# fperezgamonal/flownet2-tf

Hardware: AMD Instinct MI355X
Metric: forward pairs/sec at 512x384 (FlowNet2) (higher is better)
Workload: dtype f16x2 (split fp16 hi+lo operands, 3 fp16 MFMAs per product, fp32 accumulate); 1 GPU; FlowNet2 forward, batch=4 synthetic 512x384 pairs per GPU, seeded synthetic weights; pairs_per_gpu=4, parallelism=dp1 (no collective)

## Files before the change

### flownet2-tf_amd/csrc/corr3.hip

```cpp
#include "fn2_common.h"

namespace fn2 {

typedef __attribute__((address_space(3))) void* lptr3_t;

struct CorrArgs {
  const void* a;
  const void* b;
  void* out;
  int N, H, W;
  int a_cs, a_c0, b_cs, b_c0, out_cs, out_c0;
  int md, s2, gr, gw, lo;
  int act;
  float c_f;
};

#ifndef FN2_C3_XS
#define FN2_C3_XS 2
#endif
constexpr int C3_XS = FN2_C3_XS;
constexpr int C3_HALF = C3_XS == 2 ? 64 : 48;
constexpr int C3_ROWS = 2 * C3_HALF;
constexpr int C3_OTS = 168;
#ifndef FN2_C3_SLOTS
#define FN2_C3_SLOTS 3
#endif
constexpr int C3_SLOTS = FN2_C3_SLOTS;
constexpr int C3_SG = 1;
constexpr int C3_TY = 2;
constexpr int C3_NW = 2 * C3_TY * C3_XS;
constexpr int C3_PX = 32 * C3_TY * C3_XS;
constexpr unsigned kOob3 = 0x80000000u;

typedef int v4i3_t __attribute__((ext_vector_type(4)));

__device__ __forceinline__ void dma16_3(const v4i3_t rsrc, const void* lds, unsigned voff, int soff) {
  const unsigned la = (unsigned)(unsigned long long)(lptr3_t)lds;
  asm volatile("s_mov_b32 m0, %0\n\ts_nop 0\n\tbuffer_load_dwordx4 %1, %2, %3 offen lds"
               :: "s"(la), "v"(voff), "s"(rsrc), "s"(soff) : "memory");
}

template <typename T, typename OutT, int NL>
__global__ void __launch_bounds__(64 * C3_NW) corr3_kernel(const CorrArgs p, const int b_bytes, const int dbg) {
#if defined(__HIP_DEVICE_COMPILE__)
  constexpr int ESZ = (int)sizeof(T);
  constexpr bool X2 = is_x2<T>::value;
  constexpr int SG = NL < C3_SG ? 1 : C3_SG;
  constexpr int NST = NL / SG;
  constexpr int NPIECE = C3_ROWS * SG / 8;
  constexpr int PPW = (NPIECE + C3_NW - 1) / C3_NW;
  __shared__ uint4 ring[C3_SLOTS][C3_SG][C3_ROWS * 8];
  __shared__ float ot[C3_PX * C3_OTS];

  const int tid = threadIdx.x, lane = tid & 63;
  const int wave = __builtin_amdgcn_readfirstlane(tid >> 6);
  const int gx = gridDim.x, gy = gridDim.y;
  const int NT = gx * gy * (int)gridDim.z, L = blockIdx.x + gx * (blockIdx.y + gy * blockIdx.z);
  const int xcd = L & 7, chk = NT >> 3, rem = NT & 7;
  const int Lp = xcd * chk + min(xcd, rem) + (L >> 3);
  const int xb = (Lp % gx) * (32 * C3_XS);
  const int g = (Lp / gx) % gy;
  const int zc = Lp / (gx * gy);
  const int n = zc / 3, c = zc - n * 3;
  const int y0 = 2 * C3_TY * (g >> 1) + (g & 1);
  const int pi0 = 8 * c, npi = min(8, p.gw - pi0);

  const int fi = lane & 15, fg = lane >> 4;
  const int hh = wave % C3_XS, par = (wave / C3_XS) & 1, r = wave / (2 * C3_XS);
  const int ya = y0 + 2 * r;
  const int xa = xb + 32 * hh + par + 2 * fi;

  for (int i = tid; i < C3_PX * C3_OTS / 4; i += 64 * C3_NW) reinterpret_cast<float4*>(ot)[i] = make_float4(0.f, 0.f, 0.f, 0.f);

  uint4 fa[NL][2];
  {
    const bool ok = xa < p.W && ya < p.H;
    const char* src = reinterpret_cast<const char*>(p.a) +
                      ((((size_t)n * p.H + (ok ? ya : 0)) * p.W + (ok ? xa : 0)) * p.a_cs + p.a_c0) * ESZ;
#pragma unroll
    for (int l = 0; l < NL; ++l)
#pragma unroll
      for (int q = 0; q < 2; ++q) {
        const int chunk = X2 ? (2 * fg + q) : (4 * q + fg);
        fa[l][q] = ok ? *reinterpret_cast<const uint4*>(src + l * 128 + chunk * 16) : make_uint4(0, 0, 0, 0);
      }
  }

  const int yb0 = y0 + 2 * (pi0 - p.gr);
  int k_lo = 0, k_hi = npi + C3_TY - 2;
  while (k_lo <= k_hi && yb0 + 2 * k_lo < 0) ++k_lo;
  while (k_hi >= k_lo && yb0 + 2 * k_hi >= p.H) --k_hi;
  const int nrow = k_hi - k_lo + 1;
  const int S = nrow > 0 ? nrow * NST : 0;

  const v4i3_t rsrc = v4i3_t{(int)((unsigned long long)p.b & 0xffffffffu), (int)(((unsigned long long)p.b >> 32) & 0xffffu),
                             b_bytes, 0x00020000};
  unsigned voff[PPW];
#pragma unroll
  for (int k = 0; k < PPW; ++k) {
    const int q = wave * PPW + k;
    const int sl = q / (C3_ROWS / 8), rg = q - sl * (C3_ROWS / 8);
    const int rho = rg * 8 + (lane >> 3);
    const int Lc = (lane & 7) ^ ((rho >> 1) & 7);
    const int G = X2 ? ((Lc & 3) * 2 + (Lc >> 2)) : Lc;
    const int px = rho < C3_HALF ? 2 * rho : 2 * (rho - C3_HALF) + 1;
    const int xw = xb - p.md + px;
    const bool ok = q < NPIECE && xw >= 0 && xw < p.W;
    voff[k] = ok ? (unsigned)((xw * p.b_cs + p.b_c0) * ESZ + sl * 128 + G * 16) : kOob3;
  }
  const int row_bytes = p.W * p.b_cs * ESZ;
  int is_s = 0, is_st = 0, is_slot = 0;
  int is_soff = (n * p.H + yb0 + 2 * k_lo) * row_bytes;
  auto issue_stage = [&]() {
    uint4 (*slot)[C3_ROWS * 8] = ring[is_slot];
    const bool live = is_s < S;
#pragma unroll
    for (int k = 0; k < PPW; ++k) {
      const int q = wave * PPW + k;
      const int sl = q / (C3_ROWS / 8), rg = q - sl * (C3_ROWS / 8);
      if (q < NPIECE && !(dbg & 1)) dma16_3(rsrc, &slot[sl][rg * 64], live ? voff[k] : kOob3, live ? is_soff : 0);
    }
    ++is_s;
    is_slot = is_slot == C3_SLOTS - 1 ? 0 : is_slot + 1;
    if (++is_st == NST) { is_st = 0; is_soff += 2 * row_bytes - (NST - 1) * SG * 128; }
    else is_soff += SG * 128;
  };

  const int fsw = (fi >> 1) & 7;
  const int rbase = par * C3_HALF + 16 * hh + fi;
  const int ci = (int)p.c_f;
  const bool pow2 = (ci & (ci - 1)) == 0;
  const float rcp = 1.f / p.c_f;
  f32x4 acc[3];
#pragma unroll
  for (int tb = 0; tb < 3; ++tb) acc[tb] = f32x4{0.f, 0.f, 0.f, 0.f};

  if (S > 0) {
#pragma unroll
    for (int d = 0; d < C3_SLOTS - 1; ++d) issue_stage();
    __syncthreads();
    int cslot = 0;
    for (int kk = 0; kk < nrow; ++kk) {
#pragma unroll
      for (int st = 0; st < NST; ++st) {
        static_assert(PPW * (C3_SLOTS - 2) <= 63, "vmcnt field");
        asm volatile("s_waitcnt vmcnt(%0)\n\ts_barrier" :: "n"(PPW * (C3_SLOTS - 2)) : "memory");
        issue_stage();
        uint4 (*slot)[C3_ROWS * 8] = ring[cslot];
        cslot = cslot == C3_SLOTS - 1 ? 0 : cslot + 1;
        const int pil_s = k_lo + kk - r;
        if (!(dbg & 2) && pil_s >= 0 && pil_s < npi)
#pragma unroll
        for (int sl = 0; sl < SG; ++sl) {
          const int l = st * SG + sl;
#pragma unroll
          for (int tb = 0; tb < 3; ++tb) {
            const uint4* row = &slot[sl][(rbase + 16 * tb) * 8];
            const uint4 b0 = row[fg ^ fsw], b1 = row[(4 + fg) ^ fsw];
            if constexpr (X2) {
              acc[tb] = mfma_16x16x32<f16_t>(fa[l][1], b0, acc[tb]);
              acc[tb] = mfma_16x16x32<f16_t>(fa[l][0], b1, acc[tb]);
              acc[tb] = mfma_16x16x32<f16_t>(fa[l][0], b0, acc[tb]);
            } else {
              acc[tb] = mfma_16x16x32<T>(fa[l][0], b0, acc[tb]);
              acc[tb] = mfma_16x16x32<T>(fa[l][1], b1, acc[tb]);
            }
          }
        }
      }
      const int pil = k_lo + kk - r;
      const bool rowok = pil >= 0 && pil < npi;
#pragma unroll
      for (int tb = 0; tb < 3; ++tb) {
#pragma unroll
        for (int q = 0; q < 4; ++q) {
          const int i = fg * 4 + q;
          const int o = 16 * tb + fi - i;
          if (rowok && o >= 0 && o <= 2 * p.gr && !(dbg & 4)) {
            float v = pow2 ? acc[tb][q] * rcp : acc[tb][q] / p.c_f;
            if (p.act == FN2_ACT_LEAKY) v = leaky(v);
            ot[(r * 32 * C3_XS + 32 * hh + par + 2 * i) * C3_OTS + pil * p.gw + o] = v;
          }
        }
        acc[tb] = f32x4{0.f, 0.f, 0.f, 0.f};
      }
    }
    asm volatile("s_waitcnt vmcnt(0)" ::: "memory");
  }
  __syncthreads();

  if (dbg & 8) return;
  OutT* out = reinterpret_cast<OutT*>(p.out);
  const int nch = npi * p.gw;
  const int ch0 = p.out_c0 + pi0 * p.gw;
  if constexpr (is_x2<OutT>::value) {
    const int ngrp = nch >> 3;
    for (int idx = tid; idx < C3_PX * ngrp; idx += 64 * C3_NW) {
      const int px = idx / ngrp, gi = idx - px * ngrp;
      const int rr = px / (32 * C3_XS), x = xb + px % (32 * C3_XS), y = y0 + 2 * rr;
      if (x >= p.W || y >= p.H) continue;
      const float* src = &ot[px * C3_OTS + gi * 8];
      float v[8];
      *reinterpret_cast<float4*>(v) = *reinterpret_cast<const float4*>(src);
      *reinterpret_cast<float4*>(v + 4) = *reinterpret_cast<const float4*>(src + 4);
      uint4* q = reinterpret_cast<uint4*>(out + (((size_t)n * p.H + y) * p.W + x) * p.out_cs + ch0 + gi * 8);
      split8(v, q[0], q[1]);
    }
    const int tail = nch - (ngrp << 3);
    for (int idx = tid; idx < C3_PX * tail; idx += 64 * C3_NW) {
      const int px = idx / tail, j = (ngrp << 3) + (idx - px * tail);
      const int rr = px / (32 * C3_XS), x = xb + px % (32 * C3_XS), y = y0 + 2 * rr;
      if (x < p.W && y < p.H)
        store_elem<OutT>(out + (((size_t)n * p.H + y) * p.W + x) * p.out_cs + ch0 + j, ot[px * C3_OTS + j]);
    }
  } else {
    for (int idx = tid; idx < C3_PX * nch; idx += 64 * C3_NW) {
      const int px = idx / nch, j = idx - px * nch;
      const int rr = px / (32 * C3_XS), x = xb + px % (32 * C3_XS), y = y0 + 2 * rr;
      if (x < p.W && y < p.H)
        store_elem<OutT>(out + (((size_t)n * p.H + y) * p.W + x) * p.out_cs + ch0 + j, ot[px * C3_OTS + j]);
    }
  }
#endif
}

template <typename T, typename OutT>
static int launch3(const CorrArgs& a, int C, int b_bytes, hipStream_t s) {
  const int nl = C * (int)sizeof(T) / 128;
  dim3 grid(cdiv(a.W, 32 * C3_XS), a.H / C3_TY, a.N * 3), block(64 * C3_NW);
  const char* e_dbg = getenv("FN2_CORR3_DBG");
  const int dbg = e_dbg ? atoi(e_dbg) : 0;
  switch (nl) {
#define FN2_C3_CASE(NL_)                                                               \
  case NL_:                                                                            \
    hipLaunchKernelGGL((corr3_kernel<T, OutT, NL_>), grid, block, 0, s, a, b_bytes, dbg);   \
    break;
    FN2_C3_CASE(1)
    FN2_C3_CASE(2)
    FN2_C3_CASE(4)
    FN2_C3_CASE(8)
#undef FN2_C3_CASE
    default:
      return fail(FN2_ERR_UNSUPPORTED, "correlation: unsupported channel count %d", C);
  }
  FN2_CHECK_LAUNCH("corr3");
  return FN2_OK;
}

bool corr3_ok(int C, int in_dtype, int out_dtype, int md, int s2, int H, int out_cs, int out_c0, long b_bytes) {
  const char* e = getenv("FN2_CORR3");
  if (e && atoi(e) == 0) return false;
  if (in_dtype == FN2_F32) return false;
  const int esz = dtype_size(in_dtype);
  if ((C * esz) % 128 != 0) return false;
  const int nl = C * esz / 128;
  if (!(nl == 1 || nl == 2 || nl == 4 || nl == 8)) return false;
  if (md != 20 || s2 != 2 || H % (2 * C3_TY) != 0 || b_bytes >= (1L << 31)) return false;
  if (out_dtype == FN2_F16X2 && (out_cs % 8 != 0 || out_c0 % 8 != 0)) return false;
  return true;
}

int launch_corr3(const void* a, int a_cs, int a_c0, const void* b, int b_cs, int b_c0, void* out, int out_cs,
                 int out_c0, int in_dtype, int out_dtype, int N, int H, int W, int C, int md, int s2, int gr, int gw,
                 int act, hipStream_t s) {
  CorrArgs g;
  g.a = a; g.b = b; g.out = out;
  g.N = N; g.H = H; g.W = W;
  g.a_cs = a_cs; g.a_c0 = a_c0; g.b_cs = b_cs; g.b_c0 = b_c0; g.out_cs = out_cs; g.out_c0 = out_c0;
  g.md = md; g.s2 = s2; g.gr = gr; g.gw = gw; g.lo = md - gr * s2;
  g.act = act;
  g.c_f = (float)C;
  const int bb = (int)((long)N * H * W * b_cs * dtype_size(in_dtype));
  if (in_dtype == FN2_BF16) return out_dtype == FN2_BF16 ? launch3<bf16_t, bf16_t>(g, C, bb, s) : launch3<bf16_t, float>(g, C, bb, s);
  if (in_dtype == FN2_F16) return out_dtype == FN2_F16 ? launch3<f16_t, f16_t>(g, C, bb, s) : launch3<f16_t, float>(g, C, bb, s);
  return out_dtype == FN2_F16X2 ? launch3<x2_t, x2_t>(g, C, bb, s) : launch3<x2_t, float>(g, C, bb, s);
}

}
```

Before: 1131 pairs/s.

## Keep all correlation rows in registers and use per-wave LDS transpose epilogue

The correlation kernel now keeps accumulators for every displacement row in registers (acc[KR][3]) instead of flushing to a shared output tile after each row, and stages two channel slices per pipeline step. The shared ring and the output staging buffer are merged into one LDS array. Each wave transposes its own results through that buffer and writes them out without a block-wide barrier. Displacement radius is hardcoded to 10, and the scale and leaky branches are specialised at compile time. The aim is to cut LDS footprint, per-row epilogue work and block syncs, at the cost of much higher register pressure and reduced generality.

```diff
diff --git a/flownet2-tf_amd/csrc/corr3.hip b/flownet2-tf_amd/csrc/corr3.hip
--- a/flownet2-tf_amd/csrc/corr3.hip
+++ b/flownet2-tf_amd/csrc/corr3.hip
@@ -1,3 +1,5 @@
+#include <type_traits>
+
 #include "fn2_common.h"
 
 namespace fn2 {
@@ -15,21 +17,19 @@
   float c_f;
 };
 
-#ifndef FN2_C3_XS
-#define FN2_C3_XS 2
-#endif
-constexpr int C3_XS = FN2_C3_XS;
-constexpr int C3_HALF = C3_XS == 2 ? 64 : 48;
+constexpr int C3_XS = 2;
+constexpr int C3_HALF = 64;
 constexpr int C3_ROWS = 2 * C3_HALF;
-constexpr int C3_OTS = 168;
-#ifndef FN2_C3_SLOTS
-#define FN2_C3_SLOTS 3
-#endif
-constexpr int C3_SLOTS = FN2_C3_SLOTS;
-constexpr int C3_SG = 1;
+constexpr int C3_LINE = C3_ROWS * 8;
+constexpr int C3_GR = 10, C3_GW = 2 * C3_GR + 1;
+constexpr int C3_OTS = 8 * C3_GW;
+constexpr int C3_SLOTS = 3;
+constexpr int C3_SG = 2;
 constexpr int C3_TY = 2;
 constexpr int C3_NW = 2 * C3_TY * C3_XS;
-constexpr int C3_PX = 32 * C3_TY * C3_XS;
+constexpr int C3_KR = 8 + C3_TY - 1;
+constexpr int C3_PXS = 192, C3_ROW0 = 24;
+constexpr int C3_EPI = 16 * C3_PXS + 32;
 constexpr unsigned kOob3 = 0x80000000u;
 
 typedef int v4i3_t __attribute__((ext_vector_type(4)));
@@ -38,6 +38,11 @@
   const unsigned la = (unsigned)(unsigned long long)(lptr3_t)lds;
   asm volatile("s_mov_b32 m0, %0\n\ts_nop 0\n\tbuffer_load_dwordx4 %1, %2, %3 offen lds"
                :: "s"(la), "v"(voff), "s"(rsrc), "s"(soff) : "memory");
+}
+
+__device__ __forceinline__ float leaky_c3(float x) {
+#pragma clang fp contract(off)
+  return 0.55f * x + 0.45f * fabsf(x);
 }
 
 template <typename T, typename OutT, int NL>
@@ -45,12 +50,13 @@
 #if defined(__HIP_DEVICE_COMPILE__)
   constexpr int ESZ = (int)sizeof(T);
   constexpr bool X2 = is_x2<T>::value;
-  constexpr int SG = NL < C3_SG ? 1 : C3_SG;
+  constexpr int SG = NL < C3_SG ? NL : C3_SG;
   constexpr int NST = NL / SG;
   constexpr int NPIECE = C3_ROWS * SG / 8;
   constexpr int PPW = (NPIECE + C3_NW - 1) / C3_NW;
-  __shared__ uint4 ring[C3_SLOTS][C3_SG][C3_ROWS * 8];
-  __shared__ float ot[C3_PX * C3_OTS];
+  constexpr int RING16 = C3_SLOTS * SG * C3_LINE;
+  constexpr int EPI16 = C3_NW * C3_EPI / 4;
+  __shared__ uint4 lds[RING16 > EPI16 ? RING16 : EPI16];
 
   const int tid = threadIdx.x, lane = tid & 63;
   const int wave = __builtin_amdgcn_readfirstlane(tid >> 6);
@@ -63,14 +69,12 @@
   const int zc = Lp / (gx * gy);
   const int n = zc / 3, c = zc - n * 3;
   const int y0 = 2 * C3_TY * (g >> 1) + (g & 1);
-  const int pi0 = 8 * c, npi = min(8, p.gw - pi0);
+  const int pi0 = 8 * c, npi = min(8, C3_GW - pi0);
 
   const int fi = lane & 15, fg = lane >> 4;
   const int hh = wave % C3_XS, par = (wave / C3_XS) & 1, r = wave / (2 * C3_XS);
   const int ya = y0 + 2 * r;
   const int xa = xb + 32 * hh + par + 2 * fi;
-
-  for (int i = tid; i < C3_PX * C3_OTS / 4; i += 64 * C3_NW) reinterpret_cast<float4*>(ot)[i] = make_float4(0.f, 0.f, 0.f, 0.f);
 
   uint4 fa[NL][2];
   {
@@ -86,7 +90,7 @@
       }
   }
 
-  const int yb0 = y0 + 2 * (pi0 - p.gr);
+  const int yb0 = y0 + 2 * (pi0 - C3_GR);
   int k_lo = 0, k_hi = npi + C3_TY - 2;
   while (k_lo <= k_hi && yb0 + 2 * k_lo < 0) ++k_lo;
   while (k_hi >= k_lo && yb0 + 2 * k_hi >= p.H) --k_hi;
@@ -112,13 +116,13 @@
   int is_s = 0, is_st = 0, is_slot = 0;
   int is_soff = (n * p.H + yb0 + 2 * k_lo) * row_bytes;
   auto issue_stage = [&]() {
-    uint4 (*slot)[C3_ROWS * 8] = ring[is_slot];
+    uint4* slot = lds + is_slot * (SG * C3_LINE);
     const bool live = is_s < S;
 #pragma unroll
     for (int k = 0; k < PPW; ++k) {
       const int q = wave * PPW + k;
       const int sl = q / (C3_ROWS / 8), rg = q - sl * (C3_ROWS / 8);
-      if (q < NPIECE && !(dbg & 1)) dma16_3(rsrc, &slot[sl][rg * 64], live ? voff[k] : kOob3, live ? is_soff : 0);
+      if (q < NPIECE && !(dbg & 1)) dma16_3(rsrc, &slot[sl * C3_LINE + rg * 64], live ? voff[k] : kOob3, live ? is_soff : 0);
     }
     ++is_s;
     is_slot = is_slot == C3_SLOTS - 1 ? 0 : is_slot + 1;
@@ -128,97 +132,128 @@
 
   const int fsw = (fi >> 1) & 7;
   const int rbase = par * C3_HALF + 16 * hh + fi;
-  const int ci = (int)p.c_f;
-  const bool pow2 = (ci & (ci - 1)) == 0;
-  const float rcp = 1.f / p.c_f;
-  f32x4 acc[3];
-#pragma unroll
-  for (int tb = 0; tb < 3; ++tb) acc[tb] = f32x4{0.f, 0.f, 0.f, 0.f};
+  f32x4 acc[C3_KR][3];
+#pragma unroll
+  for (int k = 0; k < C3_KR; ++k)
+#pragma unroll
+    for (int tb = 0; tb < 3; ++tb) acc[k][tb] = f32x4{0.f, 0.f, 0.f, 0.f};
 
   if (S > 0) {
 #pragma unroll
     for (int d = 0; d < C3_SLOTS - 1; ++d) issue_stage();
-    __syncthreads();
+#pragma unroll
+    for (int l = 0; l < NL; ++l)
+#pragma unroll
+      for (int q = 0; q < 2; ++q) {
+        v4i3_t t = __builtin_bit_cast(v4i3_t, fa[l][q]);
+        asm volatile("" : "+v"(t));
+        fa[l][q] = __builtin_bit_cast(uint4, t);
+      }
     int cslot = 0;
-    for (int kk = 0; kk < nrow; ++kk) {
-#pragma unroll
-      for (int st = 0; st < NST; ++st) {
-        static_assert(PPW * (C3_SLOTS - 2) <= 63, "vmcnt field");
-        asm volatile("s_waitcnt vmcnt(%0)\n\ts_barrier" :: "n"(PPW * (C3_SLOTS - 2)) : "memory");
-        issue_stage();
-        uint4 (*slot)[C3_ROWS * 8] = ring[cslot];
-        cslot = cslot == C3_SLOTS - 1 ? 0 : cslot + 1;
-        const int pil_s = k_lo + kk - r;
-        if (!(dbg & 2) && pil_s >= 0 && pil_s < npi)
-#pragma unroll
-        for (int sl = 0; sl < SG; ++sl) {
-          const int l = st * SG + sl;
-#pragma unroll
-          for (int tb = 0; tb < 3; ++tb) {
-            const uint4* row = &slot[sl][(rbase + 16 * tb) * 8];
-            const uint4 b0 = row[fg ^ fsw], b1 = row[(4 + fg) ^ fsw];
+#pragma unroll
+    for (int k = 0; k < C3_KR; ++k) {
+      if (k >= k_lo && k <= k_hi) {
+        const int pil = k - r;
+        const bool used = !(dbg & 2) && pil >= 0 && pil < npi;
+#pragma unroll
+        for (int st = 0; st < NST; ++st) {
+          static_assert(PPW * (C3_SLOTS - 2) <= 63, "vmcnt field");
+          asm volatile("s_waitcnt vmcnt(%0)\n\ts_barrier" :: "n"(PPW * (C3_SLOTS - 2)) : "memory");
+          issue_stage();
+          const uint4* slot = lds + cslot * (SG * C3_LINE);
+          cslot = cslot == C3_SLOTS - 1 ? 0 : cslot + 1;
+          if (used)
+#pragma unroll
+          for (int sl = 0; sl < SG; ++sl) {
+            const int l = st * SG + sl;
+            uint4 b0[3], b1[3];
+#pragma unroll
+            for (int tb = 0; tb < 3; ++tb) {
+              const uint4* row = &slot[sl * C3_LINE + (rbase + 16 * tb) * 8];
+              b0[tb] = row[fg ^ fsw];
+              b1[tb] = row[(4 + fg) ^ fsw];
+            }
             if constexpr (X2) {
-              acc[tb] = mfma_16x16x32<f16_t>(fa[l][1], b0, acc[tb]);
-              acc[tb] = mfma_16x16x32<f16_t>(fa[l][0], b1, acc[tb]);
-              acc[tb] = mfma_16x16x32<f16_t>(fa[l][0], b0, acc[tb]);
+#pragma unroll
+              for (int tb = 0; tb < 3; ++tb) acc[k][tb] = mfma_16x16x32<f16_t>(fa[l][1], b0[tb], acc[k][tb]);
+#pragma unroll
+              for (int tb = 0; tb < 3; ++tb) acc[k][tb] = mfma_16x16x32<f16_t>(fa[l][0], b1[tb], acc[k][tb]);
+#pragma unroll
+              for (int tb = 0; tb < 3; ++tb) acc[k][tb] = mfma_16x16x32<f16_t>(fa[l][0], b0[tb], acc[k][tb]);
             } else {
-              acc[tb] = mfma_16x16x32<T>(fa[l][0], b0, acc[tb]);
-              acc[tb] = mfma_16x16x32<T>(fa[l][1], b1, acc[tb]);
+#pragma unroll
+              for (int tb = 0; tb < 3; ++tb) acc[k][tb] = mfma_16x16x32<T>(fa[l][0], b0[tb], acc[k][tb]);
+#pragma unroll
+              for (int tb = 0; tb < 3; ++tb) acc[k][tb] = mfma_16x16x32<T>(fa[l][1], b1[tb], acc[k][tb]);
             }
           }
         }
       }
-      const int pil = k_lo + kk - r;
-      const bool rowok = pil >= 0 && pil < npi;
-#pragma unroll
-      for (int tb = 0; tb < 3; ++tb) {
-#pragma unroll
-        for (int q = 0; q < 4; ++q) {
-          const int i = fg * 4 + q;
-          const int o = 16 * tb + fi - i;
-          if (rowok && o >= 0 && o <= 2 * p.gr && !(dbg & 4)) {
-            float v = pow2 ? acc[tb][q] * rcp : acc[tb][q] / p.c_f;
-            if (p.act == FN2_ACT_LEAKY) v = leaky(v);
-            ot[(r * 32 * C3_XS + 32 * hh + par + 2 * i) * C3_OTS + pil * p.gw + o] = v;
+    }
+    asm volatile("s_waitcnt vmcnt(0)" ::: "memory");
+    __syncthreads();
+  }
+
+  float* ow = reinterpret_cast<float*>(lds) + wave * C3_EPI;
+  auto transpose = [&](auto pow2_c, auto leaky_c) {
+    constexpr bool POW2 = decltype(pow2_c)::value, LEAKY = decltype(leaky_c)::value;
+    const float rcp = 1.f / p.c_f;
+    float* wb = ow + 4 * fg * (C3_PXS - 1) + fi + C3_ROW0 - r * C3_GW;
+#pragma unroll
+    for (int tb = 0; tb < 3; ++tb)
+#pragma unroll
+      for (int q = 0; q < 4; ++q) {
+        const int o = 16 * tb + fi - (fg * 4 + q);
+        if (o >= 0 && o <= 2 * C3_GR)
+#pragma unroll
+          for (int k = 0; k < C3_KR; ++k) {
+            float v = POW2 ? acc[k][tb][q] * rcp : acc[k][tb][q] / p.c_f;
+            if (LEAKY) v = leaky_c3(v);
+            wb[q * (C3_PXS - 1) + 16 * tb + k * C3_GW] = v;
           }
-        }
-        acc[tb] = f32x4{0.f, 0.f, 0.f, 0.f};
       }
-    }
-    asm volatile("s_waitcnt vmcnt(0)" ::: "memory");
-  }
-  __syncthreads();
+  };
+  if (!(dbg & 4)) {
+    const int ci = (int)p.c_f;
+    const bool pow2 = (ci & (ci - 1)) == 0, lk = p.act == FN2_ACT_LEAKY;
+    if (pow2) { if (lk) transpose(std::true_type{}, std::true_type{}); else transpose(std::true_type{}, std::false_type{}); }
+    else { if (lk) transpose(std::false_type{}, std::true_type{}); else transpose(std::false_type{}, std::false_type{}); }
+  }
+  __builtin_amdgcn_fence(__ATOMIC_RELEASE, "wavefront");
+  __builtin_amdgcn_wave_barrier();
+  __builtin_amdgcn_fence(__ATOMIC_ACQUIRE, "wavefront");
 
   if (dbg & 8) return;
   OutT* out = reinterpret_cast<OutT*>(p.out);
-  const int nch = npi * p.gw;
-  const int ch0 = p.out_c0 + pi0 * p.gw;
+  const int nch = npi * C3_GW;
+  const int ch0 = p.out_c0 + pi0 * C3_GW;
+  const int xs = xb + 32 * hh + par;
+  if (ya >= p.H) return;
+  OutT* orow = out + ((size_t)n * p.H + ya) * p.W * p.out_cs + ch0;
   if constexpr (is_x2<OutT>::value) {
     const int ngrp = nch >> 3;
-    for (int idx = tid; idx < C3_PX * ngrp; idx += 64 * C3_NW) {
-      const int px = idx / ngrp, gi = idx - px * ngrp;
-      const int rr = px / (32 * C3_XS), x = xb + px % (32 * C3_XS), y = y0 + 2 * rr;
-      if (x >= p.W || y >= p.H) continue;
-      const float* src = &ot[px * C3_OTS + gi * 8];
+    for (int idx = lane; idx < 16 * ngrp; idx += 64) {
+      const int i = idx / ngrp, gi = idx - i * ngrp;
+      const int x = xs + 2 * i;
+      if (x >= p.W) continue;
+      const float* src = &ow[i * C3_PXS + C3_ROW0 + gi * 8];
       float v[8];
       *reinterpret_cast<float4*>(v) = *reinterpret_cast<const float4*>(src);
       *reinterpret_cast<float4*>(v + 4) = *reinterpret_cast<const float4*>(src + 4);
-      uint4* q = reinterpret_cast<uint4*>(out + (((size_t)n * p.H + y) * p.W + x) * p.out_cs + ch0 + gi * 8);
+      uint4* q = reinterpret_cast<uint4*>(orow + (size_t)x * p.out_cs + gi * 8);
       split8(v, q[0], q[1]);
     }
     const int tail = nch - (ngrp << 3);
-    for (int idx = tid; idx < C3_PX * tail; idx += 64 * C3_NW) {
-      const int px = idx / tail, j = (ngrp << 3) + (idx - px * tail);
-      const int rr = px / (32 * C3_XS), x = xb + px % (32 * C3_XS), y = y0 + 2 * rr;
-      if (x < p.W && y < p.H)
-        store_elem<OutT>(out + (((size_t)n * p.H + y) * p.W + x) * p.out_cs + ch0 + j, ot[px * C3_OTS + j]);
+    for (int idx = lane; idx < 16 * tail; idx += 64) {
+      const int i = idx / tail, j = (ngrp << 3) + (idx - i * tail);
+      const int x = xs + 2 * i;
+      if (x < p.W) store_elem<OutT>(orow + (size_t)x * p.out_cs + j, ow[i * C3_PXS + C3_ROW0 + j]);
     }
   } else {
-    for (int idx = tid; idx < C3_PX * nch; idx += 64 * C3_NW) {
-      const int px = idx / nch, j = idx - px * nch;
-      const int rr = px / (32 * C3_XS), x = xb + px % (32 * C3_XS), y = y0 + 2 * rr;
-      if (x < p.W && y < p.H)
-        store_elem<OutT>(out + (((size_t)n * p.H + y) * p.W + x) * p.out_cs + ch0 + j, ot[px * C3_OTS + j]);
+    for (int idx = lane; idx < 16 * nch; idx += 64) {
+      const int i = idx / nch, j = idx - i * nch;
+      const int x = xs + 2 * i;
+      if (x < p.W) store_elem<OutT>(orow + (size_t)x * p.out_cs + j, ow[i * C3_PXS + C3_ROW0 + j]);
     }
   }
 #endif
```

New measurement: 1135 pairs/s (median of 6 runs). Within noise of the previous version (+0.3%).
